# ZongyueQin/SessionSimilaritySearch

Hardware: AMD Instinct MI355X
Metric: session queries/sec (higher is better)
Workload: dtype f32

## Files before the change

### sessionsimilaritysearch_amd/csrc/scan_kernel.h

```cpp
#pragma once
#include "scan.h"
#include "scan_dev.h"

#ifndef SSS_STAGGER
#define SSS_STAGGER 1
#endif
#ifndef SSS_F32_SCHED
#define SSS_F32_SCHED 7
#endif

namespace sss {

extern __device__ unsigned g_boot_expired;

template <int RB, int TR, int DT, int NW, bool THR = false, bool AP = false, int MET = 0>
__global__ __launch_bounds__(NW * 64, AP ? 2 * (NW / 4) : NW / 4) void k_scan(const ScanArgs A) {
    constexpr int H = TR / 64;
    constexpr int CH = RB / 16;
    constexpr int NU = RB / 32;
    constexpr int TILE_BYTES = TR * RB;
    constexpr int LOADS_PER_WAVE = TR * CH / 64 / NW;
    constexpr int WGQ = NW * 32;
    constexpr bool PRECOMP = RB <= 512 && !AP;
    constexpr int TAU_LDS = 2 * TILE_BYTES;
    constexpr bool F32S = (SSS_F32_SCHED & 1) && DT == DT_F32 && !AP && !THR && RB == 512;
    static_assert(CH <= 64, "row longer than one LDS-DMA instruction");
    static_assert(LOADS_PER_WAVE >= 1, "a tile is at least one DMA piece per wave");
    extern __shared__ __attribute__((aligned(16))) char smem[];

    const int nq = A.nq, n = A.n, S = A.S, G = A.G, J = A.J;
    const char* __restrict__ Qb = reinterpret_cast<const char*>(A.Q);
    const char* __restrict__ Cb = reinterpret_cast<const char*>(A.C);
    const int tid = threadIdx.x;
    const int lane = tid & 63;
    const int wave = __builtin_amdgcn_readfirstlane(tid >> 6);
    const int r = lane & 31, h = lane >> 5;

    const int bid = blockIdx.x;
    const int xcd = bid & 7, slot = bid >> 3;
    const int split = xcd * (S >> 3) + slot / G;
    const int g = slot % G;

    const int q_local = wave * 32 + r;
    const int q_glob = g * WGQ + q_local;
    int q_ld = q_glob < nq ? q_glob : nq - 1;
    if constexpr (THR) q_ld = A.qsel[q_ld];
    f32x4 qc[NU];

    float ls[KP];
    int li[KP];
#pragma unroll
    for (int i = 0; i < KP; ++i) { ls[i] = -INFINITY; li[i] = -1; }
    float pend_s = -INFINITY;
    int pend_i = -1;
    constexpr int E = 4;
    float es[E];
    int ei[E];
    int ecnt = 0;
#pragma unroll
    for (int i = 0; i < E; ++i) { es[i] = -INFINITY; ei[i] = -1; }
    float tau = -INFINITY, thr = -INFINITY;
    if constexpr (THR) thr = q_glob < nq ? A.thr[q_glob] : INFINITY;
    float rmax = -INFINITY;
    float pub = -INFINITY;

    int tile_lo = split * A.tiles_per_split;
    int tile_hi = tile_lo + A.tiles_per_split;
    if (tile_hi > A.total_tiles) tile_hi = A.total_tiles;
    const int ntiles = tile_lo < tile_hi ? tile_hi - tile_lo : 0;
    const bool use_tau = !THR && J > 0;
    const bool boot = use_tau && A.boot && ntiles > 0;
    const int nb = boot ? 1 : 0;
    const int niter = ntiles + nb;
    auto tile_of = [&](int i) { return i < ntiles ? tile_lo + i : tile_lo; };
    const int skip = A.tau_skip;

    bool slots_seen = false;
    const unsigned* my_half = nullptr;
    unsigned cls_live = 0;
#ifdef SSS_EXP_NOPAIR
    const bool pair_pub = false;
#else
    const bool pair_pub = A.cert == 1;
#endif
    if (use_tau) {
        cls_live = pair_pub ? (unsigned)(split + (split >> 4)) & 15u : (unsigned)(2 * split + h) % (unsigned)A.Ju;
        my_half = A.slots + (size_t)q_ld * SLOT_STRIDE + h * (J >> 1);
    }
    auto tau_ord = [&]() -> unsigned {
        if (J == 16 && skip > 0) {
            unsigned v[8];
            load8_sc1(my_half, v);
            return tau_select16(v, skip, h);
        }
        unsigned m = 0xFFFFFFFFu;
        for (int v = 0; v < (J >> 1); v += 8) m = min(m, min8_sc1(my_half + v));
        return min(m, (unsigned)__shfl_xor((int)m, 32));
    };
    const unsigned tau_lds = (unsigned)(unsigned long)(lptr_c)smem + TAU_LDS + wave * 2048;
    auto tau_fetch = [&]() {
        int ln = lane;
        asm volatile("" : "+v"(ln));
#pragma unroll
        for (int j = 0; j < 2; ++j) {
            int qi = g * WGQ + wave * 32 + 16 * j + (ln >> 2);
            if (qi > nq - 1) qi = nq - 1;
            const unsigned off = (unsigned)qi * (unsigned)(SLOT_STRIDE * 4) + (unsigned)(ln & 3) * 16u;
            const unsigned dst = __builtin_amdgcn_readfirstlane(tau_lds + j * 1024);
            asm volatile("s_mov_b32 m0, %1\n\ts_nop 0\n\tglobal_load_lds_dwordx4 %0, %2 sc1"
                         : : "v"(off), "s"(dst), "s"(A.slots) : "memory");
        }
    };
    auto tau_read = [&]() -> unsigned {
        const u32x4* p = reinterpret_cast<const u32x4*>(smem + TAU_LDS + wave * 2048 + r * 64 + h * 32);
        const u32x4 a = p[0], b = p[1];
        if (skip > 0) {
            unsigned v[8] = {a.x, a.y, a.z, a.w, b.x, b.y, b.z, b.w};
            return tau_select16(v, skip, h);
        }
        const unsigned m = min(min(min(a.x, a.y), min(a.z, a.w)), min(min(b.x, b.y), min(b.z, b.w)));
        return min(m, (unsigned)__shfl_xor((int)m, 32));
    };
    auto set_tau = [&](unsigned m) {
        if (m > ORD_NEG_INF) tau = fmaxf(tau, ord2f(m - 1));
        thr = AP ? tau : fmaxf(ls[KP - 1], tau);
    };
    auto publish = [&](unsigned cls) {
        float val = rmax;
        bool ok = true;
        if (A.cert > 1) {
            float v2 = ls[1], v4 = ls[3], v8 = ls[7], v16 = ls[KP - 1];
            int i2 = li[1], i4 = li[3], i8 = li[7], i16 = li[KP - 1];
            asm volatile("" : "+v"(v2), "+v"(v4), "+v"(v8), "+v"(v16), "+v"(i2), "+v"(i4), "+v"(i8), "+v"(i16));
            const int c = A.cert;
            val = c == 2 ? v2 : c == 4 ? v4 : c == 8 ? v8 : v16;
            ok = (c == 2 ? i2 : c == 4 ? i4 : c == 8 ? i8 : i16) >= 0;
        }
        if (pair_pub) { val = fmaxf(val, __shfl_xor(val, 32)); ok = h == 0; }
        unsigned cur = 0u;
        if (J == 16 && slots_seen) cur = *reinterpret_cast<const unsigned*>(smem + TAU_LDS + wave * 2048 + r * 64 + cls * 4u);
        if (ok && val > pub && val > tau && f2ord(val) > cur && q_glob < nq) {
            int qq = THR ? q_ld : q_glob;
            asm volatile("" : "+v"(qq));
            __hip_atomic_fetch_max(A.slots + ((size_t)(unsigned)qq * (unsigned)SLOT_STRIDE + cls), f2ord(val), __ATOMIC_RELAXED, __HIP_MEMORY_SCOPE_AGENT);
            pub = val;
        }
    };

    const unsigned lds_base = (unsigned)(unsigned long)(lptr_c)smem;
    auto slot_row = [&](int i) { return ((wave * LOADS_PER_WAVE + i) * 64 + lane) / CH; };
    auto slot_off = [&](int i) {
        const int p = (wave * LOADS_PER_WAVE + i) * 64 + lane;
        const int tr = p / CH, sc = p % CH;
        return (unsigned)(tr * RB + ((sc ^ (tr & 15)) * 16));
    };
    unsigned lane_off[PRECOMP ? LOADS_PER_WAVE : 1];
    if (PRECOMP) {
#pragma unroll
        for (int i = 0; i < LOADS_PER_WAVE; ++i) lane_off[i] = slot_off(i);
    }
    auto stage_piece = [&](int buf, int tile_idx, int i) {
        const long row0 = (long)tile_idx * TR;
        const bool inside = row0 + TR <= (long)n;
        const char* tile_src = Cb + (size_t)row0 * RB;
        const unsigned dst = __builtin_amdgcn_readfirstlane(
            lds_base + buf * TILE_BYTES + (wave * LOADS_PER_WAVE + i) * 1024);
        unsigned off = PRECOMP ? lane_off[PRECOMP ? i : 0] : slot_off(i);
        if (!inside) {
            const int lr = slot_row(i);
            long grow = row0 + lr;
            if (grow > (long)n - 1) grow = (long)n - 1;
            off = (unsigned)((grow - row0) * RB) + (off - (unsigned)(lr * RB));
        }
        asm volatile("s_mov_b32 m0, %1\n\ts_nop 0\n\tglobal_load_lds_dwordx4 %0, %2"
                     : : "v"(off), "s"(dst), "s"(tile_src) : "memory");
    };
    auto stage = [&](int buf, int tile_idx) {
#pragma unroll
        for (int i = 0; i < LOADS_PER_WAVE; ++i) stage_piece(buf, tile_idx, i);
    };

    const int x = h ^ (r & 15);
    f32x16 acc0 = {0}, acc1 = {0};
    [[maybe_unused]] float bcur[MET ? 2 * H : 1];
    [[maybe_unused]] float bscale = 1.f;
    [[maybe_unused]] auto bias_fetch = [&](int tile_idx) {
#pragma unroll
        for (int s = 0; s < 2 * H; ++s) {
            long row = (long)tile_idx * TR + s * 32 + r;
            if (row > (long)n - 1) row = (long)n - 1;
            bcur[s] = h == 0 ? A.bias[row] : 0.f;
        }
    };
    [[maybe_unused]] auto bias_land = [&]() {
#pragma unroll
        for (int s = 0; s < 2 * H; ++s) asm volatile("" : "+v"(bcur[s]));
    };

    auto mfma_sub = [&](int buf, int sub, int next_tile) {
        const char* tile = smem + buf * TILE_BYTES + sub * (64 * RB);
        if constexpr (H == 1) { if (next_tile >= 0) stage(buf ^ 1, next_tile); }
        auto lda = [&](int u) -> const f32x4* {
            const int c = (2 * u) ^ x;
            return reinterpret_cast<const f32x4*>(tile + (r * CH + c) * 16);
        };
        constexpr int PF = DT == DT_F32 ? 1 : AP ? 1 : (RB == 256 ? NU : RB == 512 ? 4 : 2);
        f32x4 as0[NU], as1[NU];
#pragma unroll
        for (int u = 0; u < PF && u < NU; ++u) { const f32x4* p = lda(u); as0[u] = p[0]; as1[u] = p[32 * CH]; }
        const f32x16 zero = {0};
        if constexpr (MET) {
            float b0 = bcur[0], b1 = bcur[1];
#pragma unroll
            for (int s = 1; s < H; ++s) { b0 = sub == s ? bcur[2 * s] : b0; b1 = sub == s ? bcur[2 * s + 1] : b1; }
            acc0 = __builtin_amdgcn_mfma_f32_32x32x2f32(b0, bscale, zero, 0, 0, 0);
            acc1 = __builtin_amdgcn_mfma_f32_32x32x2f32(b1, bscale, zero, 0, 0, 0);
        } else {
            acc0 = zero; acc1 = zero;
        }
        [[maybe_unused]] i32x16 ia0 = {0}, ia1 = {0};
#pragma unroll
        for (int u = 0; u < NU; ++u) {
            if (u + PF < NU) { const f32x4* p = lda(u + PF); as0[u + PF] = p[0]; as1[u + PF] = p[32 * CH]; }
            const f32x4 a0 = as0[u], a1 = as1[u];
            __builtin_amdgcn_sched_barrier(0);
            if constexpr (DT == DT_F32) {
                acc0 = __builtin_amdgcn_mfma_f32_32x32x2f32(a0.x, qc[u].x, acc0, 0, 0, 0);
                acc1 = __builtin_amdgcn_mfma_f32_32x32x2f32(a1.x, qc[u].x, acc1, 0, 0, 0);
                acc0 = __builtin_amdgcn_mfma_f32_32x32x2f32(a0.y, qc[u].y, acc0, 0, 0, 0);
                acc1 = __builtin_amdgcn_mfma_f32_32x32x2f32(a1.y, qc[u].y, acc1, 0, 0, 0);
                acc0 = __builtin_amdgcn_mfma_f32_32x32x2f32(a0.z, qc[u].z, acc0, 0, 0, 0);
                acc1 = __builtin_amdgcn_mfma_f32_32x32x2f32(a1.z, qc[u].z, acc1, 0, 0, 0);
                acc0 = __builtin_amdgcn_mfma_f32_32x32x2f32(a0.w, qc[u].w, acc0, 0, 0, 0);
                acc1 = __builtin_amdgcn_mfma_f32_32x32x2f32(a1.w, qc[u].w, acc1, 0, 0, 0);
            } else if constexpr (DT == DT_BF16) {
                const bf16x8 qb = __builtin_bit_cast(bf16x8, qc[u]);
                acc0 = __builtin_amdgcn_mfma_f32_32x32x16_bf16(__builtin_bit_cast(bf16x8, a0), qb, acc0, 0, 0, 0);
                acc1 = __builtin_amdgcn_mfma_f32_32x32x16_bf16(__builtin_bit_cast(bf16x8, a1), qb, acc1, 0, 0, 0);
            } else if constexpr (DT == DT_F16 || DT == DT_H16) {
                const f16x8 qb = __builtin_bit_cast(f16x8, qc[u]);
                acc0 = __builtin_amdgcn_mfma_f32_32x32x16_f16(__builtin_bit_cast(f16x8, a0), qb, acc0, 0, 0, 0);
                acc1 = __builtin_amdgcn_mfma_f32_32x32x16_f16(__builtin_bit_cast(f16x8, a1), qb, acc1, 0, 0, 0);
            } else if constexpr (DT == DT_I8) {
                const i32x4 qb = __builtin_bit_cast(i32x4, qc[u]);
                ia0 = __builtin_amdgcn_mfma_i32_32x32x32_i8(__builtin_bit_cast(i32x4, a0), qb, ia0, 0, 0, 0);
                ia1 = __builtin_amdgcn_mfma_i32_32x32x32_i8(__builtin_bit_cast(i32x4, a1), qb, ia1, 0, 0, 0);
            } else {
                const bf16x8 A0 = __builtin_bit_cast(bf16x8, a0), A1 = __builtin_bit_cast(bf16x8, a1);
                const bf16x8 qh = __builtin_bit_cast(bf16x8, qc[u < NU / 2 ? u : u - NU / 2]);
                acc0 = __builtin_amdgcn_mfma_f32_32x32x16_bf16(A0, qh, acc0, 0, 0, 0);
                acc1 = __builtin_amdgcn_mfma_f32_32x32x16_bf16(A1, qh, acc1, 0, 0, 0);
                if (u < NU / 2) {
                    const bf16x8 ql = __builtin_bit_cast(bf16x8, qc[u + NU / 2]);
                    acc0 = __builtin_amdgcn_mfma_f32_32x32x16_bf16(A0, ql, acc0, 0, 0, 0);
                    acc1 = __builtin_amdgcn_mfma_f32_32x32x16_bf16(A1, ql, acc1, 0, 0, 0);
                }
            }
            __builtin_amdgcn_sched_barrier(0);
        }
        if constexpr (DT == DT_I8) {
            acc0 = __builtin_convertvector(ia0, f32x16);
            acc1 = __builtin_convertvector(ia1, f32x16);
        }
        if constexpr (H > 1) { if (sub == 0 && next_tile >= 0) stage(buf ^ 1, next_tile); }
    };

    auto block_max = [&](const f32x16& a, float& q0, float& q1, float& q2, float& q3) {
        q0 = fmaxf(fmaxf(a[0], a[1]), fmaxf(a[2], a[3]));
        q1 = fmaxf(fmaxf(a[4], a[5]), fmaxf(a[6], a[7]));
        q2 = fmaxf(fmaxf(a[8], a[9]), fmaxf(a[10], a[11]));
        q3 = fmaxf(fmaxf(a[12], a[13]), fmaxf(a[14], a[15]));
        return fmaxf(fmaxf(q0, q1), fmaxf(q2, q3));
    };
    auto insert_block = [&](const f32x16& a, int base) {
        float q0, q1, q2, q3;
        const float m = block_max(a, q0, q1, q2, q3);
        if (__builtin_amdgcn_ballot_w64(m > thr) == 0) return;
        auto walk = [&](float qm, int j0) {
            if (__builtin_amdgcn_ballot_w64(qm > thr) == 0) return;
#pragma unroll
            for (int jj = 0; jj < 4; ++jj) {
                const int j = j0 + jj;
                const bool pass = a[j] > thr;
                if (__builtin_amdgcn_ballot_w64(pass) != 0) {
                    if (__builtin_amdgcn_ballot_w64(pass && pend_i >= 0) != 0) {
                        list_insert<KP>(ls, li, pend_s, pend_i);
                        pend_s = -INFINITY; pend_i = -1;
                        thr = fmaxf(ls[KP - 1], tau);
                    }
                    const bool still = a[j] > thr;
                    pend_s = still ? a[j] : pend_s;
                    pend_i = still ? base + (j & 3) + 8 * (j >> 2) : pend_i;
                }
            }
        };
        walk(q0, 0); walk(q1, 4); walk(q2, 8); walk(q3, 12);
    };
    auto flush = [&](bool need) {
        if (need && q_glob < nq) {
            const unsigned at = atomicAdd(A.cnt + q_glob, (unsigned)ecnt);
            unsigned long long* dst = A.cand + (size_t)q_glob * A.cap;
            unsigned long long lost = 0ull;
#pragma unroll
            for (int i = 0; i < E; ++i) {
                if (i < ecnt) {
                    const unsigned long long key = make_key(es[i], ei[i]);
                    if (at + (unsigned)i < (unsigned)A.cap) dst[at + i] = key;
                    else lost = lost > key ? lost : key;
                }
            }
            if (lost != 0ull && A.maxlast != nullptr) atomicMax(A.maxlast + q_glob, lost);
        }
        ecnt = need ? 0 : ecnt;
    };
    auto append_block = [&](const f32x16& a, int base) {
        float q0, q1, q2, q3;
        const float m = block_max(a, q0, q1, q2, q3);
        if (__builtin_amdgcn_ballot_w64(m > thr) == 0) return;
        auto walk = [&](float qm, int j0) {
            if (__builtin_amdgcn_ballot_w64(qm > thr) == 0) return;
#pragma unroll
            for (int jj = 0; jj < 4; ++jj) {
                const int j = j0 + jj;
                const bool pass = a[j] > thr;
                if (__builtin_amdgcn_ballot_w64(pass) != 0) {
                    const bool full = pass && ecnt == E;
                    if (__builtin_amdgcn_ballot_w64(full) != 0) flush(full);
#pragma unroll
                    for (int i = E - 1; i > 0; --i) { es[i] = pass ? es[i - 1] : es[i]; ei[i] = pass ? ei[i - 1] : ei[i]; }
                    es[0] = pass ? a[j] : es[0];
                    ei[0] = pass ? base + (j & 3) + 8 * (j >> 2) : ei[0];
                    ecnt += pass ? 1 : 0;
                }
            }
        };
        walk(q0, 0); walk(q1, 4); walk(q2, 8); walk(q3, 12);
    };
    auto emit_block = [&](const f32x16& a, int base) {
        float q0, q1, q2, q3;
        const float m = block_max(a, q0, q1, q2, q3);
        if (__builtin_amdgcn_ballot_w64(m > thr) == 0) return;
#pragma unroll
        for (int j = 0; j < 16; ++j) {
            if (a[j] > thr) {
                const unsigned pos = atomicAdd(A.cnt + q_glob, 1u);
                if (pos < (unsigned)A.cap) A.cand[(size_t)q_glob * A.cap + pos] = make_key(a[j], base + (j & 3) + 8 * (j >> 2));
            }
        }
    };
    const bool two_ahead = H > 1 && niter > 1;
    if (ntiles > 0) stage(0, tile_lo);
    if (two_ahead) stage(1, tile_of(1));
    if constexpr (MET) {
        int q_shift = 0;
        load_queries<RB, DT>(Qb, q_ld, h, qc, &q_shift);
        if constexpr (DT == DT_F16) {
            const int e = A.corpus_shift + q_shift;
            bscale = ldexpf(1.f, e < -126 ? -126 : e > 127 ? 127 : e);
        }
        bias_fetch(tile_of(0));
    } else {
        load_queries<RB, DT>(Qb, q_ld, h, qc);
    }
    asm volatile("s_waitcnt vmcnt(0)" ::: "memory");
    __syncthreads();
    if constexpr (MET) bias_land();

    const int T = niter * H;
    long row0_of_step = 0;
    constexpr bool TAU_EVERY_TILE = TR >= 512;
    auto refresh_at = [&](int i) {
        if (i == 1 && boot && !TAU_EVERY_TILE) return false;
        if (TAU_EVERY_TILE || i <= 4) return true;
        const int sh = 30 - __builtin_clz(i);
        return (i & ((1 << sh) - 1)) == 0;
    };
    auto tile_top = [&](int i) {
        if (!use_tau || i == 0) return;
        if (J == 16) {
            if (!refresh_at(i)) return;
            publish(cls_live);
            tau_fetch();
            return;
        }
        const int ii = i - (wave >= 4 ? 1 : 0);
        if (ii >= 2 && (ii <= 8 || (ii & (ii - 1)) == 0 || (ii & 15) == 0)) set_tau(tau_ord());
        publish(cls_live);
    };
    auto tile_end = [&](int i) {
        const bool pre = boot && i == 0;
        if (pre) publish(cls_live);
        if constexpr (MET) { if (i + 1 < niter) bias_fetch(tile_of(i + 1)); }
        asm volatile("s_waitcnt vmcnt(0)" ::: "memory");
        if (use_tau && J == 16 && i > 0 && refresh_at(i)) { set_tau(tau_read()); slots_seen = true; }
        __syncthreads();
        if (pre) {
            unsigned m = 0;
            for (int it = 0; it < (AP ? 1024 : 24); ++it) {
                m = tau_ord();
                if (__builtin_amdgcn_ballot_w64(m == 0) == 0) break;
                __builtin_amdgcn_s_sleep(16);
            }
            if constexpr (!MET) {
                if (lane == 0 && __builtin_amdgcn_ballot_w64(m == 0 && q_glob < nq) != 0) atomicAdd(&g_boot_expired, 1u);
            }
            set_tau(m);
        }
        if constexpr (MET) bias_land();
    };
    auto score_mfma = [&](int t) {
        const int i = (int)((unsigned)t / (unsigned)H), sub = (int)((unsigned)t % (unsigned)H);
        if (sub == 0) tile_top(i);
        const int next_tile = (i + 1 < niter && !(two_ahead && i == 0)) ? tile_of(i + 1) : -1;
        mfma_sub(i & 1, sub, next_tile);
        row0_of_step = (long)tile_of(i) * TR + sub * 64;
        if (row0_of_step + 64 > n) {
#pragma unroll
            for (int j = 0; j < 16; ++j) {
                const int rr = (int)row0_of_step + 4 * h + (j & 3) + 8 * (j >> 2);
                if (rr >= n) acc0[j] = -INFINITY;
                if (rr + 32 >= n) acc1[j] = -INFINITY;
            }
        }
    };
    auto score_tree = [&]() -> float {
        float m0 = vmax3(acc0[0], acc0[1], acc0[2]), m1 = vmax3(acc1[0], acc1[1], acc1[2]);
#pragma unroll
        for (int j = 3; j < 15; j += 2) { m0 = vmax3(m0, acc0[j], acc0[j + 1]); m1 = vmax3(m1, acc1[j], acc1[j + 1]); }
        const float m = vmax3(m0, m1, acc0[15]);
        const float mm = vmax3(m, acc1[15], rmax);
        rmax = mm;
        return vmax3(m, acc1[15], acc1[15]);
    };
    const int t_live = nb * H;
    const bool defer = SSS_STAGGER && NW == 8 && (DT == DT_SPLIT || DT == DT_BF16 || DT == DT_H16 || DT == DT_I8) && wave >= 4;
    int t = 0;
    if constexpr (AP || THR) {
        t = T;
        for (int i = 0; i < niter; ++i) {
            tile_top(i);
            const int tile = tile_of(i);
            const int next_tile = (i + 1 < niter && !(two_ahead && i == 0)) ? tile_of(i + 1) : -1;
            const int row_base = tile * TR;
            const bool ragged = row_base + TR > n;
            const bool live = i >= nb;
            if constexpr (THR) {
                if (g * WGQ + wave * 32 >= nq) {
                    if (next_tile >= 0) stage((i & 1) ^ 1, next_tile);
                    tile_end(i);
                    continue;
                }
            }
#pragma unroll
            for (int sub = 0; sub < H; ++sub) {
                mfma_sub(i & 1, sub, next_tile);
                const int row0 = row_base + sub * 64;
                if (ragged) {
#pragma unroll
                    for (int j = 0; j < 16; ++j) {
                        const int rr = row0 + 4 * h + (j & 3) + 8 * (j >> 2);
                        if (rr >= n) acc0[j] = -INFINITY;
                        if (rr + 32 >= n) acc1[j] = -INFINITY;
                    }
                }
                const float m = score_tree();
                if (live && __builtin_amdgcn_ballot_w64(m > thr) != 0) {
                    append_block(acc0, row0 + 4 * h);
                    append_block(acc1, row0 + 32 + 4 * h);
                }
            }
            tile_end(i);
        }
    }
    if constexpr (F32S) {
        constexpr bool SPREAD = (SSS_F32_SCHED & 2) != 0, EARLY_TREE = (SSS_F32_SCHED & 4) != 0;
        static_assert(LOADS_PER_WAVE + 1 < NU, "a DMA piece per k-group, behind k-groups 1 .. LOADS_PER_WAVE");
        const unsigned frag_lane = (unsigned)(r * CH) * 16u;
        f32x4 nf0 = {0}, nf1 = {0};
        auto frag_ptr = [&](unsigned step_off, int u) -> const f32x4* {
            const int c = (2 * u) ^ x;
            return reinterpret_cast<const f32x4*>(smem + step_off + frag_lane + c * 16);
        };
        auto read_first = [&](unsigned step_off) { const f32x4* p = frag_ptr(step_off, 0); nf0 = p[0]; nf1 = p[32 * CH]; };
        float tm0 = -INFINITY;
        auto step = [&](int t) -> float {
            const int i = (int)((unsigned)t / (unsigned)H), sub = (int)((unsigned)t % (unsigned)H);
            const unsigned off = (unsigned)((i & 1) * TILE_BYTES + sub * (64 * RB));
            f32x4 as0[NU], as1[NU];
            as0[0] = nf0; as1[0] = nf1;
            const f32x16 zero = {0};
            if constexpr (MET) {
                float b0 = bcur[0], b1 = bcur[1];
#pragma unroll
                for (int s = 1; s < H; ++s) { b0 = sub == s ? bcur[2 * s] : b0; b1 = sub == s ? bcur[2 * s + 1] : b1; }
                acc0 = __builtin_amdgcn_mfma_f32_32x32x2f32(b0, bscale, zero, 0, 0, 0);
                acc1 = __builtin_amdgcn_mfma_f32_32x32x2f32(b1, bscale, zero, 0, 0, 0);
            } else {
                acc0 = zero; acc1 = zero;
            }
            auto fetch = [&](int u) { const f32x4* p = frag_ptr(off, u); as0[u] = p[0]; as1[u] = p[32 * CH]; };
            auto mfma8 = [&](int u) {
                const f32x4 a0 = as0[u], a1 = as1[u];
                __builtin_amdgcn_sched_barrier(0);
                acc0 = __builtin_amdgcn_mfma_f32_32x32x2f32(a0.x, qc[u].x, acc0, 0, 0, 0);
                acc1 = __builtin_amdgcn_mfma_f32_32x32x2f32(a1.x, qc[u].x, acc1, 0, 0, 0);
                acc0 = __builtin_amdgcn_mfma_f32_32x32x2f32(a0.y, qc[u].y, acc0, 0, 0, 0);
                acc1 = __builtin_amdgcn_mfma_f32_32x32x2f32(a1.y, qc[u].y, acc1, 0, 0, 0);
                acc0 = __builtin_amdgcn_mfma_f32_32x32x2f32(a0.z, qc[u].z, acc0, 0, 0, 0);
                acc1 = __builtin_amdgcn_mfma_f32_32x32x2f32(a1.z, qc[u].z, acc1, 0, 0, 0);
                acc0 = __builtin_amdgcn_mfma_f32_32x32x2f32(a0.w, qc[u].w, acc0, 0, 0, 0);
                acc1 = __builtin_amdgcn_mfma_f32_32x32x2f32(a1.w, qc[u].w, acc1, 0, 0, 0);
                __builtin_amdgcn_sched_barrier(0);
            };
            fetch(1);
            mfma8(0);
            if (sub == 0) tile_top(i);
            const int next_tile = (sub == 0 && i + 1 < niter && !(two_ahead && i == 0)) ? tile_of(i + 1) : -1;
            const long nrow0 = (long)next_tile * TR;
            const bool dma_plain = next_tile >= 0 && nrow0 + TR <= (long)n;
            const char* dma_src = Cb + (size_t)nrow0 * RB;
            const unsigned dma_dst = __builtin_amdgcn_readfirstlane(lds_base + ((i & 1) ^ 1) * TILE_BYTES + wave * LOADS_PER_WAVE * 1024);
            row0_of_step = (long)tile_of(i) * TR + sub * 64;
            const bool ragged_step = row0_of_step + 64 > n;
            const bool ends_tile = sub == H - 1 && !(boot && i == 0);
            if (next_tile >= 0 && (!dma_plain || !SPREAD)) stage((i & 1) ^ 1, next_tile);
#pragma unroll
            for (int u = 1; u < NU - 1; ++u) {
                fetch(u + 1);
                mfma8(u);
                if constexpr (SPREAD) {
                    if (u <= LOADS_PER_WAVE && dma_plain)
                        asm volatile("s_mov_b32 m0, %1\n\ts_nop 0\n\tglobal_load_lds_dwordx4 %0, %2"
                                     : : "v"(lane_off[u - 1]), "s"(dma_dst + (u - 1) * 1024), "s"(dma_src) : "memory");
                }
            }
            constexpr int u = NU - 1;
            if (ends_tile) {
                asm volatile("" : "+v"(as0[u]), "+v"(as1[u]));
                tile_end(i);
            }
            if (t + 1 < T && (sub < H - 1 || ends_tile))
                read_first(sub == H - 1 ? (unsigned)(((i + 1) & 1) * TILE_BYTES) : off + 64 * RB);
            if constexpr (!EARLY_TREE) {
                mfma8(u);
            } else {
                const f32x4 a0 = as0[u], a1 = as1[u];
                __builtin_amdgcn_sched_barrier(0);
                acc0 = __builtin_amdgcn_mfma_f32_32x32x2f32(a0.x, qc[u].x, acc0, 0, 0, 0);
                acc0 = __builtin_amdgcn_mfma_f32_32x32x2f32(a0.y, qc[u].y, acc0, 0, 0, 0);
                acc0 = __builtin_amdgcn_mfma_f32_32x32x2f32(a0.z, qc[u].z, acc0, 0, 0, 0);
                acc0 = __builtin_amdgcn_mfma_f32_32x32x2f32(a0.w, qc[u].w, acc0, 0, 0, 0);
                __builtin_amdgcn_sched_barrier(0);
                acc1 = __builtin_amdgcn_mfma_f32_32x32x2f32(a1.x, qc[u].x, acc1, 0, 0, 0);
                acc1 = __builtin_amdgcn_mfma_f32_32x32x2f32(a1.y, qc[u].y, acc1, 0, 0, 0);
                __builtin_amdgcn_sched_barrier(0);
                if (ragged_step) {
#pragma unroll
                    for (int j = 0; j < 16; ++j)
                        if ((int)row0_of_step + 4 * h + (j & 3) + 8 * (j >> 2) >= n) acc0[j] = -INFINITY;
                }
                tm0 = vmax3(acc0[0], acc0[1], acc0[2]);
#pragma unroll
                for (int j = 3; j < 15; j += 2) tm0 = vmax3(tm0, acc0[j], acc0[j + 1]);
                __builtin_amdgcn_sched_barrier(0);
                acc1 = __builtin_amdgcn_mfma_f32_32x32x2f32(a1.z, qc[u].z, acc1, 0, 0, 0);
                acc1 = __builtin_amdgcn_mfma_f32_32x32x2f32(a1.w, qc[u].w, acc1, 0, 0, 0);
                __builtin_amdgcn_sched_barrier(0);
            }
            if (ragged_step) {
#pragma unroll
                for (int j = 0; j < 16; ++j) {
                    const int rr = (int)row0_of_step + 4 * h + (j & 3) + 8 * (j >> 2);
                    if (!EARLY_TREE && rr >= n) acc0[j] = -INFINITY;
                    if (rr + 32 >= n) acc1[j] = -INFINITY;
                }
            }
            if constexpr (!EARLY_TREE) return score_tree();
            float m1 = vmax3_settled(acc1[0], acc1[1], acc1[2]);
#pragma unroll
            for (int j = 3; j < 15; j += 2) m1 = vmax3(m1, acc1[j], acc1[j + 1]);
            const float m = vmax3(tm0, m1, acc0[15]);
            rmax = vmax3(m, acc1[15], rmax);
            return vmax3(m, acc1[15], acc1[15]);
        };
        if (T > 0) read_first(0);
        while (t < T) {
            bool rare = false;
            for (; t < T; ++t) {
                const float m = step(t);
                if (t < t_live) {
                    if (t == t_live - 1) {
                        tile_end(0);
                        if (t + 1 < T) read_first((unsigned)TILE_BYTES);
                    }
                    continue;
                }
                if (__builtin_amdgcn_ballot_w64(m > thr) != 0) { rare = true; break; }
            }
            if (!rare) break;
            insert_block(acc0, (int)row0_of_step + 4 * h);
            insert_block(acc1, (int)row0_of_step + 32 + 4 * h);
            ++t;
        }
    }
    while (!F32S && t < T) {
        bool rare = false;
        for (; t < T; ++t) {
            const bool last = (unsigned)t % (unsigned)H == H - 1;
            const bool early = defer && t >= t_live;
            score_mfma(t);
            if (early && last) tile_end((int)((unsigned)t / (unsigned)H));
            const float m = score_tree();
            if (t >= t_live && __builtin_amdgcn_ballot_w64(m > thr) != 0) { rare = true; break; }
            if (!early && last) tile_end((int)((unsigned)t / (unsigned)H));
        }
        if (!rare) break;
        if constexpr (THR) {
            emit_block(acc0, (int)row0_of_step + 4 * h);
            emit_block(acc1, (int)row0_of_step + 32 + 4 * h);
        } else if constexpr (AP) {
            append_block(acc0, (int)row0_of_step + 4 * h);
            append_block(acc1, (int)row0_of_step + 32 + 4 * h);
        } else {
            insert_block(acc0, (int)row0_of_step + 4 * h);
            insert_block(acc1, (int)row0_of_step + 32 + 4 * h);
        }
        if (!defer && (unsigned)t % (unsigned)H == H - 1) tile_end((int)((unsigned)t / (unsigned)H));
        ++t;
    }
    if constexpr (THR) { flush(ecnt > 0); return; }
    if constexpr (AP) flush(ecnt > 0);
    list_insert<KP>(ls, li, pend_s, pend_i);
    if (!AP && q_glob < nq) {
        int nreal = 0;
#pragma unroll
        for (int i = 0; i < KP; ++i) nreal += li[i] >= 0 ? 1 : 0;
        if (nreal > 0) {
            const unsigned base = atomicAdd(A.cnt + q_glob, (unsigned)nreal);
            unsigned long long* dst = A.cand + (size_t)q_glob * A.cap + base;
#pragma unroll
            for (int i = 0; i < KP; ++i)
                if (i < nreal) dst[i] = make_key(ls[i], li[i]);
            if (nreal == KP) atomicMax(A.maxlast + q_glob, (unsigned long long)make_key(ls[KP - 1], li[KP - 1]));
        }
    }
}

template <int RB, int TR, int DT, int NW, int MET, bool THR, bool AP = false>
static int launch_form(const ScanArgs& a, hipStream_t st) {
    const size_t lds = 2 * (size_t)TR * RB + NW * 2048;
    const int rc = opt_in_lds(reinterpret_cast<const void*>(&k_scan<RB, TR, DT, NW, THR, AP, MET>), "k_scan", lds);
    if (rc) return rc;
    hipLaunchKernelGGL((k_scan<RB, TR, DT, NW, THR, AP, MET>), dim3(a.S * a.G), dim3(NW * 64), lds, st, a);
    return check_launch("k_scan");
}
template <int RB, int TR, int DT, int NW, int MET>
static int launch_one(const ScanArgs& a, hipStream_t st) {
    if (a.thr != nullptr) {
        if constexpr (TR == (RB <= 512 ? 128 : 64)) return launch_form<RB, TR, DT, NW, MET, true>(a, st);
        set_error("scan: threshold form not built for %d-row tiles of %d-byte rows", TR, RB);
        return SSS_EINVAL;
    }
    if (a.append) {
        if constexpr (RB == 256 && TR == 128 && DT != DT_F32) return launch_form<RB, TR, DT, NW, MET, false, true>(a, st);
        set_error("scan: append form not built for this shape");
        return SSS_EINVAL;
    }
    return launch_form<RB, TR, DT, NW, MET, false>(a, st);
}
template <int DT, int MET>
static int launch_shape(int rb, int tile_rows, const ScanArgs& a, hipStream_t st) {
    if (rb == 256) return tile_rows == 256 ? launch_one<256, 256, DT, 8, MET>(a, st) : launch_one<256, 128, DT, 8, MET>(a, st);
    if (rb == 512) return tile_rows == 128 ? launch_one<512, 128, DT, 8, MET>(a, st) : launch_one<512, 64, DT, 8, MET>(a, st);
    if (rb == 1024) return launch_one<1024, 64, DT, 4, MET>(a, st);
    return 1;
}

}
```

Before: 497,100.

## Skew f32 scan steps so acc1 reduction overlaps next step's first MFMAs

```diff
diff --git a/sessionsimilaritysearch_amd/csrc/scan_kernel.h b/sessionsimilaritysearch_amd/csrc/scan_kernel.h
--- a/sessionsimilaritysearch_amd/csrc/scan_kernel.h
+++ b/sessionsimilaritysearch_amd/csrc/scan_kernel.h
@@ -1,4 +1,5 @@
 #pragma once
+#include <type_traits>
 #include "scan.h"
 #include "scan_dev.h"
 
@@ -6,7 +7,7 @@
 #define SSS_STAGGER 1
 #endif
 #ifndef SSS_F32_SCHED
-#define SSS_F32_SCHED 7
+#define SSS_F32_SCHED 15
 #endif
 
 namespace sss {
@@ -473,17 +474,54 @@
         }
     }
     if constexpr (F32S) {
-        constexpr bool SPREAD = (SSS_F32_SCHED & 2) != 0, EARLY_TREE = (SSS_F32_SCHED & 4) != 0;
+        constexpr bool SPREAD = (SSS_F32_SCHED & 2) != 0, EARLY_TREE = (SSS_F32_SCHED & 4) != 0, SKEW = (SSS_F32_SCHED & 8) != 0;
+        static_assert(!SKEW || EARLY_TREE, "bit 3 carries bit 2 across the step boundary");
         static_assert(LOADS_PER_WAVE + 1 < NU, "a DMA piece per k-group, behind k-groups 1 .. LOADS_PER_WAVE");
         const unsigned frag_lane = (unsigned)(r * CH) * 16u;
         f32x4 nf0 = {0}, nf1 = {0};
+        [[maybe_unused]] float nb0 = 0.f;
         auto frag_ptr = [&](unsigned step_off, int u) -> const f32x4* {
             const int c = (2 * u) ^ x;
             return reinterpret_cast<const f32x4*>(smem + step_off + frag_lane + c * 16);
         };
-        auto read_first = [&](unsigned step_off) { const f32x4* p = frag_ptr(step_off, 0); nf0 = p[0]; nf1 = p[32 * CH]; };
+        auto read_first = [&](unsigned step_off, [[maybe_unused]] int nsub) {
+            const f32x4* p = frag_ptr(step_off, 0); nf0 = p[0]; nf1 = p[32 * CH];
+            if constexpr (MET && SKEW) {
+                nb0 = bcur[0];
+#pragma unroll
+                for (int s = 1; s < H; ++s) nb0 = nsub == s ? bcur[2 * s] : nb0;
+            }
+        };
         float tm0 = -INFINITY;
-        auto step = [&](int t) -> float {
+        bool hit = false;
+        auto head = [&]() {
+            const f32x4 a0 = nf0;
+            const f32x16 zero = {0};
+            const bool ragged_prev = row0_of_step + 64 > n;
+            __builtin_amdgcn_sched_barrier(0);
+            if constexpr (MET) acc0 = __builtin_amdgcn_mfma_f32_32x32x2f32(nb0, bscale, zero, 0, 0, 0);
+            else acc0 = zero;
+            acc0 = __builtin_amdgcn_mfma_f32_32x32x2f32(a0.x, qc[0].x, acc0, 0, 0, 0);
+            acc0 = __builtin_amdgcn_mfma_f32_32x32x2f32(a0.y, qc[0].y, acc0, 0, 0, 0);
+            __builtin_amdgcn_sched_barrier(0);
+            if (ragged_prev) {
+#pragma unroll
+                for (int j = 0; j < 16; ++j)
+                    if ((int)row0_of_step + 32 + 4 * h + (j & 3) + 8 * (j >> 2) >= n) acc1[j] = -INFINITY;
+            }
+            float m1 = vmax3(acc1[0], acc1[1], acc1[2]);
+#pragma unroll
+            for (int j = 3; j < 15; j += 2) m1 = vmax3(m1, acc1[j], acc1[j + 1]);
+            rmax = vmax3(m1, acc1[15], rmax);
+            m1 = vmax3(m1, acc1[15], acc1[15]);
+            hit = __builtin_amdgcn_ballot_w64(m1 > thr) != 0;
+            __builtin_amdgcn_sched_barrier(0);
+            acc0 = __builtin_amdgcn_mfma_f32_32x32x2f32(a0.z, qc[0].z, acc0, 0, 0, 0);
+            acc0 = __builtin_amdgcn_mfma_f32_32x32x2f32(a0.w, qc[0].w, acc0, 0, 0, 0);
+            __builtin_amdgcn_sched_barrier(0);
+        };
+        auto step = [&](int t, auto tail_c) -> float {
+            constexpr bool TAIL = decltype(tail_c)::value;
             const int i = (int)((unsigned)t / (unsigned)H), sub = (int)((unsigned)t % (unsigned)H);
             const unsigned off = (unsigned)((i & 1) * TILE_BYTES + sub * (64 * RB));
             f32x4 as0[NU], as1[NU];
@@ -493,10 +531,11 @@
                 float b0 = bcur[0], b1 = bcur[1];
 #pragma unroll
                 for (int s = 1; s < H; ++s) { b0 = sub == s ? bcur[2 * s] : b0; b1 = sub == s ? bcur[2 * s + 1] : b1; }
-                acc0 = __builtin_amdgcn_mfma_f32_32x32x2f32(b0, bscale, zero, 0, 0, 0);
+                if constexpr (!TAIL) acc0 = __builtin_amdgcn_mfma_f32_32x32x2f32(b0, bscale, zero, 0, 0, 0);
                 acc1 = __builtin_amdgcn_mfma_f32_32x32x2f32(b1, bscale, zero, 0, 0, 0);
             } else {
-                acc0 = zero; acc1 = zero;
+                if constexpr (!TAIL) acc0 = zero;
+                acc1 = zero;
             }
             auto fetch = [&](int u) { const f32x4* p = frag_ptr(off, u); as0[u] = p[0]; as1[u] = p[32 * CH]; };
             auto mfma8 = [&](int u) {
@@ -513,7 +552,17 @@
                 __builtin_amdgcn_sched_barrier(0);
             };
             fetch(1);
-            mfma8(0);
+            if constexpr (!TAIL) {
+                mfma8(0);
+            } else {
+                const f32x4 a1 = as1[0];
+                __builtin_amdgcn_sched_barrier(0);
+                acc1 = __builtin_amdgcn_mfma_f32_32x32x2f32(a1.x, qc[0].x, acc1, 0, 0, 0);
+                acc1 = __builtin_amdgcn_mfma_f32_32x32x2f32(a1.y, qc[0].y, acc1, 0, 0, 0);
+                acc1 = __builtin_amdgcn_mfma_f32_32x32x2f32(a1.z, qc[0].z, acc1, 0, 0, 0);
+                acc1 = __builtin_amdgcn_mfma_f32_32x32x2f32(a1.w, qc[0].w, acc1, 0, 0, 0);
+                __builtin_amdgcn_sched_barrier(0);
+            }
             if (sub == 0) tile_top(i);
             const int next_tile = (sub == 0 && i + 1 < niter && !(two_ahead && i == 0)) ? tile_of(i + 1) : -1;
             const long nrow0 = (long)next_tile * TR;
@@ -540,7 +589,7 @@
                 tile_end(i);
             }
             if (t + 1 < T && (sub < H - 1 || ends_tile))
-                read_first(sub == H - 1 ? (unsigned)(((i + 1) & 1) * TILE_BYTES) : off + 64 * RB);
+                read_first(sub == H - 1 ? (unsigned)(((i + 1) & 1) * TILE_BYTES) : off + 64 * RB, sub == H - 1 ? 0 : sub + 1);
             if constexpr (!EARLY_TREE) {
                 mfma8(u);
             } else {
@@ -562,10 +611,15 @@
                 tm0 = vmax3(acc0[0], acc0[1], acc0[2]);
 #pragma unroll
                 for (int j = 3; j < 15; j += 2) tm0 = vmax3(tm0, acc0[j], acc0[j + 1]);
+                if constexpr (TAIL) {
+                    rmax = vmax3(tm0, acc0[15], rmax);
+                    hit = __builtin_amdgcn_ballot_w64(vmax3(tm0, acc0[15], acc0[15]) > thr) != 0;
+                }
                 __builtin_amdgcn_sched_barrier(0);
                 acc1 = __builtin_amdgcn_mfma_f32_32x32x2f32(a1.z, qc[u].z, acc1, 0, 0, 0);
                 acc1 = __builtin_amdgcn_mfma_f32_32x32x2f32(a1.w, qc[u].w, acc1, 0, 0, 0);
                 __builtin_amdgcn_sched_barrier(0);
+                if constexpr (TAIL) return 0.f;
             }
             if (ragged_step) {
 #pragma unroll
@@ -583,24 +637,69 @@
             rmax = vmax3(m, acc1[15], rmax);
             return vmax3(m, acc1[15], acc1[15]);
         };
-        if (T > 0) read_first(0);
-        while (t < T) {
-            bool rare = false;
-            for (; t < T; ++t) {
-                const float m = step(t);
-                if (t < t_live) {
-                    if (t == t_live - 1) {
-                        tile_end(0);
-                        if (t + 1 < T) read_first((unsigned)TILE_BYTES);
+        constexpr std::false_type whole{};
+        if constexpr ((SSS_F32_SCHED & 16) != 0) {
+            if (wave >= 4) __builtin_amdgcn_s_setprio(1);
+        }
+        if (T > 0) read_first(0, 0);
+        if constexpr (SKEW) {
+            constexpr std::true_type tail{};
+            for (; t < t_live; ++t) {
+                step(t, whole);
+                if (t == t_live - 1) {
+                    tile_end(0);
+                    if (t + 1 < T) read_first((unsigned)TILE_BYTES, 0);
+                }
+            }
+            if (t < T) {
+#pragma unroll
+                for (int j = 0; j < 16; ++j) acc1[j] = -INFINITY;
+                head();
+                for (;;) {
+                    int rare = 0;
+                    for (;;) {
+                        step(t, tail);
+                        ++t;
+                        if (hit) { rare = 2; break; }
+                        if (t == T) break;
+                        head();
+                        if (hit) { rare = 1; break; }
                     }
-                    continue;
-                }
-                if (__builtin_amdgcn_ballot_w64(m > thr) != 0) { rare = true; break; }
-            }
-            if (!rare) break;
-            insert_block(acc0, (int)row0_of_step + 4 * h);
-            insert_block(acc1, (int)row0_of_step + 32 + 4 * h);
-            ++t;
+                    if (rare == 2) {
+                        insert_block(acc0, (int)row0_of_step + 4 * h);
+                        if (t == T) break;
+                        head();
+                        if (hit) rare = 1;
+                    }
+                    if (rare == 1) insert_block(acc1, (int)row0_of_step + 32 + 4 * h);
+                    if (t == T) break;
+                }
+                if (row0_of_step + 64 > n) {
+#pragma unroll
+                    for (int j = 0; j < 16; ++j)
+                        if ((int)row0_of_step + 32 + 4 * h + (j & 3) + 8 * (j >> 2) >= n) acc1[j] = -INFINITY;
+                }
+                insert_block(acc1, (int)row0_of_step + 32 + 4 * h);
+            }
+        } else {
+            while (t < T) {
+                bool rare = false;
+                for (; t < T; ++t) {
+                    const float m = step(t, whole);
+                    if (t < t_live) {
+                        if (t == t_live - 1) {
+                            tile_end(0);
+                            if (t + 1 < T) read_first((unsigned)TILE_BYTES, 0);
+                        }
+                        continue;
+                    }
+                    if (__builtin_amdgcn_ballot_w64(m > thr) != 0) { rare = true; break; }
+                }
+                if (!rare) break;
+                insert_block(acc0, (int)row0_of_step + 4 * h);
+                insert_block(acc1, (int)row0_of_step + 32 + 4 * h);
+                ++t;
+            }
         }
     }
     while (!F32S && t < T) {
```

After: 505,000, median of 6. 1.6% higher.
